# baggepinnen/LPVSpectral.jl

Measured on AMD Instinct MI355X. Metric: signals/sec, ls_sparse_spectral_lpv group lasso N=2^20 Nf=512 Nv=8 (2000 ADMM iters; iters/sec in admm_iters_per_sec), higher is better.
Workload: dtype f64

## Files before the change

### lpvspectral.jl_amd/csrc/api.hip

```cpp
#include <cmath>
#include <cstdarg>
#include <cstdio>
#include <cstdlib>
#include <cstring>
#include <ctime>
#include <map>
#include <mutex>
#include <array>
#include <thread>
#include <string>
#include <vector>

#include "lpvs_internal.h"

namespace lpvs {

static thread_local char g_err[512] = "";

void set_error(const char *fmt, ...) {
    va_list ap;
    va_start(ap, fmt);
    vsnprintf(g_err, sizeof(g_err), fmt, ap);
    va_end(ap);
}
// ... 448 lines not shown

AdmmParams make_params(const lpvs_problem *h) {
    const StoragePlan &pl = h->plan;
    const bool sym = h->np >= kSymmetricMinNp;
    AdmmParams p{h->M.as<double>(), h->np, h->n, h->bs.as<double>(), h->x.as<double>(), h->z.as<double>(), h->u.as<double>(),
                 h->rhs.as<double>(), h->mu, h->tol, h->prox_kind, h->prox_param, h->group_len, h->status.as<AdmmStatus>(),
                 h->scratch.as<double>(), h->part.as<double>(), sym ? h->Mp.as<double>() : nullptr, (int)h->ns};
    p.mp_f32 = pl.mode == kMpF32 ? 1 : 0;
    p.mp_split = pl.mode == kMpSplit || pl.mode == kMpMixed ? 1 : 0;
    p.mp_types = pl.mode == kMpMixed ? mp_tile_types(h->Mp, h->np, 1) : nullptr;
    p.mp_fix32 = p.mp_types != nullptr && (pl.fix_bits <= 32 || pl.nib_period > 0) ? 1 : 0;
    p.nib_period = pl.nib_period; p.nib_ramp = pl.nib_ramp; p.xb_corr = h->xb_corr.as<double>(); p.nib_rhs = h->nib_rhs.as<double>(); p.nib_part = h->nib_part.as<double>(); p.nib_acc = h->nib_acc.as<long long>();
    p.xb = pl.offset_form ? h->xb.as<double>() : nullptr;
    p.fi = pl.owns_fi && h->fi.p ? h->fi.as<double>() : nullptr;
    p.fi_R = h->fi_R; p.fi_xbmax = h->fi_xbmax;
    p.fi_prefetch_all = pl.mode == kMpMixed && h->Mp_census.fixed == h->Mp_census.total ? 1 : 0;
    p.opt_iteration = h->opt[LPVS_OPT_ITERATION]; p.opt_nt_loads = h->opt[LPVS_OPT_NT_LOADS];
    {
        const char *e = experiment_env("LPVS_TILE_ORDER");
        p.tile_order = p.fi != nullptr && !(e && std::string(e) == "forward") ? 1 : 0;
    }
    p.sm_ctl = !sym && h->sm_ctl.p ? h->sm_ctl.as<int>() : nullptr;
    p.prox_params = h->prox_per_signal && h->ns > 1 ? h->prox_params.as<double>() : nullptr;
    return p;
}

int32_t factorize(lpvs_problem *h, double shift) {
    if (h->M_valid && h->M_shift == shift) return LPVS_OK;
    const int64_t np = h->np, n = h->n;
    h->Mp_valid = false; h->Mp_rowsum = 0;
    if (!h->M.p) LPVS_TRY(h->M.alloc(sizeof(double) * (size_t)np * (size_t)np));
    if (!h->work.p) LPVS_TRY(h->work.alloc(spd_inverse_work_bytes(np)));
    LPVS_HIP(hipEventRecord(h->ev[3].a, h->stream));
    LPVS_HIP(hipMemcpyAsync(h->M.p, h->G.p, sizeof(double) * (size_t)np * (size_t)np, hipMemcpyDeviceToDevice, h->stream));
    LPVS_TRY(launch_add_diag(h->M.as<double>(), np, n, shift, h->stream));
    LPVS_TRY(spd_inverse_inplace(h->M.as<double>(), np, h->work.as<double>(), h->istat.as<int>(), h->stream, &h->res->aux));
    LPVS_HIP(hipEventRecord(h->ev[3].b, h->stream));
    int st = 0;
    LPVS_HIP(hipMemcpyAsync(&st, h->istat.p, sizeof(int), hipMemcpyDeviceToHost, h->stream));
    LPVS_HIP(hipStreamSynchronize(h->stream));
    h->t_factor += h->ev[3].ms();
    if (st != 0) {
        h->M_valid = false;
        set_error("(G + %.3g I) is not positive definite (non-positive pivot in the block sweep)", shift);
        return LPVS_ENUMERIC;
    }
    h->M_valid = true; h->M_shift = shift;
    return LPVS_OK;
}


StoragePlan decide_plan(lpvs_problem *h) {
    const int xc_opt = option_in_effect(LPVS_OPT_XUPDATE_CORRECTION, h->opt[LPVS_OPT_XUPDATE_CORRECTION]);
    const bool corrected = h->np >= kSymmetricMinNp && xc_opt != LPVS_XCORR_OFF;
    h->xcorr = xcorr_schedule_from(corrected ? experiment_env("LPVS_XUPDATE_CORRECTION") : nullptr, xcorr_default_schedule(h->ns, corrected));
    const int storage = option_in_effect(LPVS_OPT_M_STORAGE, h->opt[LPVS_OPT_M_STORAGE]);
    return admm_storage_plan(h->np, h->ns, h->f32, storage, h->ns > 1 && multi_signal_fixed_tiles_ok(h->np), h->xcorr.on(), fix_bits_from(experiment_env),
                             nib_knobs_from(experiment_env));
}

int32_t pack_mixed(lpvs_problem *h, const StoragePlan &want, StoragePlan *stored) {
    hipStream_t s = h->stream;
    const PackedLayout lay = packed_layout(h->np, want.element_bytes, 1);
    unsigned char *types = mp_tile_types(h->Mp, h->np, 1);
    unsigned long long *amax = reinterpret_cast<unsigned long long *>(h->Mp.as<unsigned char>() + lay.absmax_off);
    LPVS_TRY(launch_pack_tiles_mixed(h->M.as<double>(), h->np, h->Mp.as<unsigned char>(), types, amax, s, want.diag_float,
                                     want.want_rowsum ? h->part.as<double>() : nullptr, h->n, want.want_rowsum ? h->scratch.as<double>() : nullptr, want.fix_bits));
    std::vector<unsigned char> ht(lay.tiles);
// ... 2786 lines not shown
```

### lpvspectral.jl_amd/csrc/linalg.hip

```cpp
#include "lpvs_internal.h"
#include "factor_plan.h"

#include <cstdlib>
#include <map>
#include <mutex>
#include <string>
#include <vector>

namespace lpvs {

namespace {

typedef double f64x4 __attribute__((ext_vector_type(4)));
constexpr int NB = 64;

__global__ void __launch_bounds__(256)
diag_inverse_kernel(const double *__restrict__ Aall, int64_t np, int k, double *__restrict__ Pall, int *status,
                    int64_t strideA, int64_t strideW) {
    __shared__ double colp[NB], rowp[NB];
    const double *A = Aall + (int64_t)blockIdx.x * strideA;
    double *P = Pall + (int64_t)blockIdx.x * strideW;
    const double *blk = A + (int64_t)k * NB * np + (int64_t)k * NB;
    const int ti = threadIdx.x >> 4, tj = threadIdx.x & 15;
    double v[4][4];
#pragma unroll
    for (int a = 0; a < 4; ++a)
#pragma unroll
        for (int b = 0; b < 4; ++b) {
            const int i = 4 * ti + a, j = 4 * tj + b;
            v[a][b] = j <= i ? blk[(int64_t)i * np + j] : blk[(int64_t)j * np + i];
        }
    for (int pb = 0; pb < NB / 4; ++pb) {
#pragma unroll
        for (int pp = 0; pp < 4; ++pp) {
// ... 623 lines not shown
            S[li * KWF + (c ^ (2 * li))] = acc[b][rg];
        }
    __syncthreads();
#pragma unroll
    for (int i = 0; i < KWF * RS / 256; ++i) {
        const int e = tid + 256 * i, r = e >> 7, c = e & 127;
        A[(R0 + r) * np + k0 + c] = S[r * KWF + (c ^ (2 * r))];
    }
}

constexpr int kMaxGroup = 4;
struct RuGroup {
    const double *Ck[kMaxGroup], *Bk[kMaxGroup];
    int kb, mg;
};
template <int BK, int WGS>
__global__ void __launch_bounds__(RU_THREADS, WGS)
rank_updatem_kernel(double *__restrict__ A, int64_t np, int64_t ldp, RuGroup g, const int2 *__restrict__ tiles, int ntiles,
                    int select, int e0, int nslices, int band, int skip0, int nskip) {
    extern __shared__ __attribute__((aligned(16))) double lds[];
    const int tid = threadIdx.x, lane = tid & 63;
    const int wave = __builtin_amdgcn_readfirstlane(tid >> 6);
    const int wa = wave / RU_WN, wb = wave % RU_WN;
    int2 tt;
    if (select == 1) {
        const int nr = (int)(np / RU_TM);
        const int bsl = blockIdx.x / nr, e = blockIdx.x - bsl * nr, bt = e0 + bsl;
        if (e > bt && e < e0 + nslices) return;
        tt = e <= bt ? make_int2(bt, e) : make_int2(e, bt);
    } else {
        const int bq = ntiles / 8, br = ntiles % 8, xcd = blockIdx.x % 8, bm = blockIdx.x / 8;
        const int item = (xcd < br ? xcd * (bq + 1) : br * (bq + 1) + (xcd - br) * bq) + bm;
        tt = tiles[item];
        if ((tt.x >= skip0 && tt.x < skip0 + nskip) || (tt.y >= skip0 && tt.y < skip0 + nskip)) return;
    }
    const int jr = (tt.x >= g.kb && tt.x < g.kb + g.mg) ? tt.x - g.kb : -1, jc = (tt.y >= g.kb && tt.y < g.kb + g.mg) ? tt.y - g.kb : -1;
    int lo, hi;
    if (band >= 0) { lo = (jc >= 0 && jc < band) ? jc + 1 : 0; hi = band; }
    else { lo = (jr > jc ? jr : jc) + 1; hi = g.mg; }
    if (lo >= hi) return;
    const int64_t a0 = (int64_t)tt.x * RU_TM, b0 = (int64_t)tt.y * RU_TN;
    const int64_t r_lo = a0 + wa * 64, c_lo = b0 + wb * 64;
    const bool skip_wave = c_lo > r_lo + 63 || c_lo >= np;
    constexpr int SPP = 128 / BK;
    const int nstages = (hi - lo) * SPP;

    constexpr int ROW = RU_TM + RU_TN, STAGE = BK * ROW;
    double *buf0 = lds, *buf1 = lds + STAGE;
    auto stage_load = [&](double *buf, int st) {
        const int pi = lo + st / SPP, s0 = (st % SPP) * BK;
        const double *Ck = nullptr, *Bk = nullptr;
#pragma unroll
        for (int i = 0; i < kMaxGroup; ++i) if (i == pi) { Ck = g.Ck[i]; Bk = g.Bk[i]; }
        for (int p = wave; p < BK * 2; p += RU_THREADS / 64) {
            const int k = p >> 1, part = p & 1;
            const double *src = part == 0 ? Ck + (int64_t)(s0 + k) * ldp + a0 : Bk + (int64_t)(s0 + k) * ldp + b0;
            glds16(src + 2 * lane, buf + p * 128);
        }
    };
    const int li = lane & 15, lk = lane >> 4;
    int offA[4], offB[4];
#pragma unroll
    for (int t = 0; t < 4; ++t) { offA[t] = wa * 64 + t * 16 + li; offB[t] = RU_TM + wb * 64 + t * 16 + li; }
    stage_load(buf0, 0);
    f64x4 acc[4][4];
    const unsigned voffb = (unsigned)((lk * np + li) * 8);
    const bool below = c_lo + 63 <= r_lo;
    if (!skip_wave && below) {
#pragma unroll
        for (int i = 0; i < 4; ++i)
#pragma unroll
            for (int r = 0; r < 4; ++r) {
// ... 49 lines not shown
        for (int i = 0; i < 4; ++i)
#pragma unroll
            for (int r = 0; r < 4; ++r) {
                double *sp = A + (r_lo + i * 16 + 4 * r) * np + c_lo;
#pragma unroll
                for (int j = 0; j < 4; ++j) *reinterpret_cast<double *>(reinterpret_cast<char *>(sp + j * 16) + voffb) = acc[i][j][r];
            }
        return;
    }
#pragma unroll
    for (int i = 0; i < 4; ++i)
#pragma unroll
        for (int j = 0; j < 4; ++j)
#pragma unroll
            for (int r = 0; r < 4; ++r) {
                const int64_t row = r_lo + i * 16 + lk + 4 * r, col = c_lo + j * 16 + li;
                if (col <= row) A[row * np + col] = acc[i][j][r];
            }
}

template <int BK>
__global__ void __launch_bounds__(256, 4)
rank_updateb_kernel(double *__restrict__ A, int64_t np, int64_t ldp, RuGroup g, int e0, int nslices, int band) {
    extern __shared__ __attribute__((aligned(16))) double lds[];
    const int tid = threadIdx.x, lane = tid & 63;
    const int wave = __builtin_amdgcn_readfirstlane(tid >> 6);
    const int wa = wave >> 1, wb = wave & 1;
    const int sub = blockIdx.x & 3, bidx = blockIdx.x >> 2, sx = sub >> 1, sy = sub & 1;
    const int nr = (int)(np / 128);
    const int bsl = bidx / nr, e = bidx - bsl * nr, bt = e0 + bsl;
    if (e > bt && e < e0 + nslices) return;
    const int2 tt = e <= bt ? make_int2(bt, e) : make_int2(e, bt);
    if (tt.x == tt.y && sy > sx) return;
    const int jr = (tt.x >= g.kb && tt.x < g.kb + g.mg) ? tt.x - g.kb : -1, jc = (tt.y >= g.kb && tt.y < g.kb + g.mg) ? tt.y - g.kb : -1;
    int lo, hi;
    if (band >= 0) { lo = (jc >= 0 && jc < band) ? jc + 1 : 0; hi = band; }
    else { lo = (jr > jc ? jr : jc) + 1; hi = g.mg; }
    if (lo >= hi) return;
    const int64_t a0 = (int64_t)tt.x * 128 + sx * 64, b0 = (int64_t)tt.y * 128 + sy * 64;
    const int64_t r_lo = a0 + wa * 32, c_lo = b0 + wb * 32;
    const bool skip_wave = c_lo > r_lo + 31;
    constexpr int SPP = 128 / BK;
    const int nstages = (hi - lo) * SPP;
    constexpr int ROW = 128, STAGE = BK * ROW;
    double *buf0 = lds, *buf1 = lds + STAGE;
    auto stage_load = [&](double *buf, int st) {
        const int pi = lo + st / SPP, s0 = (st % SPP) * BK;
        const double *Ck = nullptr, *Bk = nullptr;
#pragma unroll
        for (int i = 0; i < kMaxGroup; ++i) if (i == pi) { Ck = g.Ck[i]; Bk = g.Bk[i]; }
        for (int k = wave; k < BK; k += 4) {
            const double *src = lane < 32 ? Ck + (int64_t)(s0 + k) * ldp + a0 + 2 * lane : Bk + (int64_t)(s0 + k) * ldp + b0 + 2 * (lane - 32);
            glds16(src, buf + k * ROW);
        }
    };
    const int li = lane & 15, lk = lane >> 4;
    int offA[2], offB[2];
#pragma unroll
    for (int t = 0; t < 2; ++t) { offA[t] = wa * 32 + t * 16 + li; offB[t] = 64 + wb * 32 + t * 16 + li; }
    stage_load(buf0, 0);
    f64x4 acc[2][2];
    const unsigned voffb = (unsigned)((lk * np + li) * 8);
    const bool below = c_lo + 31 <= r_lo;
    if (!skip_wave && below) {
#pragma unroll
        for (int i = 0; i < 2; ++i)
#pragma unroll
            for (int r = 0; r < 4; ++r) {
                const double *sp = A + (r_lo + i * 16 + 4 * r) * np + c_lo;
#pragma unroll
// ... 38 lines not shown
                        acc[i][j] = __builtin_amdgcn_mfma_f64_16x16x4f64(opA[i], opB[j], acc[i][j], 0, 0, 0);
                __builtin_amdgcn_sched_barrier(0);
            }
        }
        __syncthreads();
    }
    if (skip_wave) return;
    if (below) {
#pragma unroll
        for (int i = 0; i < 2; ++i)
#pragma unroll
            for (int r = 0; r < 4; ++r) {
                double *sp = A + (r_lo + i * 16 + 4 * r) * np + c_lo;
#pragma unroll
                for (int j = 0; j < 2; ++j) *reinterpret_cast<double *>(reinterpret_cast<char *>(sp + j * 16) + voffb) = acc[i][j][r];
            }
        return;
    }
#pragma unroll
    for (int i = 0; i < 2; ++i)
#pragma unroll
        for (int j = 0; j < 2; ++j)
#pragma unroll
            for (int r = 0; r < 4; ++r) {
                const int64_t row = r_lo + i * 16 + lk + 4 * r, col = c_lo + j * 16 + li;
                if (col <= row) A[row * np + col] = acc[i][j][r];
            }
}

__global__ void __launch_bounds__(256) add_diag_kernel(double *__restrict__ Mall, int64_t np, int64_t n, double shift) {
    const int64_t i = (int64_t)blockIdx.x * 256 + threadIdx.x;
    double *M = Mall + (int64_t)blockIdx.y * np * np;
    if (i < np) M[i * np + i] = i < n ? M[i * np + i] + shift : 1.0;
}

__global__ void __launch_bounds__(256) negate_mirror_kernel(double *__restrict__ Aall, int64_t np) {
    __shared__ double tile[32][33];
    double *A = Aall + (int64_t)blockIdx.z * np * np;
    const int bi = blockIdx.y, bj = blockIdx.x;
    if (bj > bi) return;
    const int tx = threadIdx.x & 31, ty = threadIdx.x >> 5;
    const int64_t r0 = (int64_t)bi * 32, c0 = (int64_t)bj * 32;
    for (int r = ty; r < 32; r += 8) {
        const double v = -A[(r0 + r) * np + c0 + tx];
        tile[r][tx] = v;
        if (bi != bj || tx <= r) A[(r0 + r) * np + c0 + tx] = v;
    }
    __syncthreads();
    for (int r = ty; r < 32; r += 8)
        if (bi != bj || tx > r) A[(c0 + r) * np + r0 + tx] = tile[tx][r];
}

__global__ void __launch_bounds__(256)
symm_matmul_kernel(const double *__restrict__ A, const double *__restrict__ B, double *__restrict__ C, int64_t np) {
    const int lane = threadIdx.x & 63, wave = threadIdx.x >> 6;
    const int64_t r0 = ((int64_t)blockIdx.y * 2 + (wave >> 1)) * 64, c0 = ((int64_t)blockIdx.x * 2 + (wave & 1)) * 64;
    const int li = lane & 15, lk = lane >> 4;
    f64x4 acc[4][4];
#pragma unroll
    for (int i = 0; i < 4; ++i)
#pragma unroll
        for (int j = 0; j < 4; ++j) acc[i][j] = (f64x4){0.0, 0.0, 0.0, 0.0};
    for (int64_t kk = 0; kk < np; kk += 4) {
        double opA[4], opB[4];
#pragma unroll
        for (int q = 0; q < 4; ++q) {
// ... 37 lines not shown
        if (two > d) d = two;
    }
    return sizeof(double) * d;
}

static void sweep64(double *A, int64_t np, int nbatch, double *work, int *status_dev, hipStream_t s) {
    const int64_t strideW = (int64_t)sweep64_work_doubles(np), strideA = np * np;
    double *Bp = work, *Cp = work + np * NB, *P = work + 2 * np * NB;
    const int nblk = (int)(np / NB);
    const int nt = (int)(np / 128);
    const unsigned ntiles = (unsigned)(nt * (nt + 1) / 2);
    for (int k = 0; k < nblk; ++k) {
        hipLaunchKernelGGL(diag_inverse_kernel, dim3((unsigned)nbatch), dim3(256), 0, s, A, np, k, P, status_dev, strideA, strideW);
        hipLaunchKernelGGL(panel_kernel, dim3((unsigned)nblk, (unsigned)nbatch), dim3(256), 0, s, A, np, k, P, Bp, Cp, strideA, strideW);
        hipLaunchKernelGGL(sweep_update_kernel, dim3(ntiles, (unsigned)nbatch), dim3(256), 0, s, A, np, k, Bp, Cp, strideA, strideW);
    }
}

static const std::vector<int2> &ru_tiles(int64_t np) {
    static std::mutex mu;
    static std::map<int64_t, std::vector<int2>> cache;
    std::lock_guard<std::mutex> g(mu);
    auto it = cache.find(np);
    if (it != cache.end()) return it->second;
    std::vector<int2> t;
    const int nr = (int)(np / RU_TM), nc = (int)ceil_div(np, RU_TN);
    for (int band = 0; band < nr; band += 4)
        for (int tj = 0; tj < nc; ++tj)
            for (int ti = band; ti < band + 4 && ti < nr; ++ti)
                if ((int64_t)tj * RU_TN <= (int64_t)ti * RU_TM + RU_TM - 1) t.push_back(make_int2(ti, tj));
    return cache.emplace(np, std::move(t)).first->second;
}

int32_t SweepAux::ensure() {
    if (side) return LPVS_OK;
    int lo = 0, hi = 0;
    LPVS_HIP(hipDeviceGetStreamPriorityRange(&lo, &hi));
    LPVS_HIP(hipStreamCreateWithPriority(&side, hipStreamNonBlocking, hi));
    LPVS_HIP(hipEventCreateWithFlags(&panel, hipEventDisableTiming));
    LPVS_HIP(hipEventCreateWithFlags(&rest, hipEventDisableTiming));
    LPVS_HIP(hipEventCreateWithFlags(&band, hipEventDisableTiming));
    LPVS_HIP(hipEventCreateWithFlags(&second, hipEventDisableTiming));
    LPVS_HIP(hipEventCreateWithFlags(&bulkdone, hipEventDisableTiming));
    const int o_res = option_in_effect(LPVS_OPT_RESERVE_CUS);
    const int reserve = o_res == LPVS_RESERVE_NONE ? 0 : (o_res > 0 ? o_res : 8);
    int dev = 0, cus = 0;
    if (reserve > 0 && hipGetDevice(&dev) == hipSuccess && hipDeviceGetAttribute(&cus, hipDeviceAttributeMultiprocessorCount, dev) == hipSuccess &&
        cus > 4 * reserve) {
        std::vector<uint32_t> mask((size_t)(cus + 31) / 32, 0u);
        for (int c = reserve; c < cus; ++c) mask[(size_t)c / 32] |= 1u << (c % 32);
        if (hipExtStreamCreateWithCUMask(&bulk, (uint32_t)mask.size(), mask.data()) != hipSuccess) { (void)hipGetLastError(); bulk = nullptr; }
    }
    return LPVS_OK;
}
SweepAux::~SweepAux() {
    if (side) { (void)hipStreamSynchronize(side); (void)hipStreamDestroy(side); }
    if (bulk) { (void)hipStreamSynchronize(bulk); (void)hipStreamDestroy(bulk); }
    if (bulkdone) (void)hipEventDestroy(bulkdone);
    if (panel) (void)hipEventDestroy(panel);
    if (rest) (void)hipEventDestroy(rest);
    if (band) (void)hipEventDestroy(band);
    if (second) (void)hipEventDestroy(second);
}


struct FactorCtx {
    double *A;
    int64_t np, ldp;
    double *panels, *P, *inner;
    int2 *tiles;
    int ntiles;
    int *status_dev;
    hipStream_t s;
    SweepAux *aux;
    double *stepB(int i) const { return panels + i * kStepPairRows * ldp; }
    double *stepC(int i) const { return stepB(i) + KW * ldp; }
    double *slotB(int blk) const { return panels + (int64_t)(blk & (kGroupSlots - 1)) * (kGroupSlotRows * ldp); }
    double *slotC(int blk) const { return slotB(blk) + 128 * ldp; }
};

constexpr size_t kRuLds = sizeof(double) * 2 * RU_BK * (RU_TM + RU_TN);

static int step_width(const FactorCtx &c, const FactorPlan &plan, int64_t k0) {
    return (int)(c.np - k0 < plan.kw_outer ? c.np - k0 : plan.kw_outer);
}

static void step_chain(const FactorCtx &c, const FactorPlan &plan, int64_t k0, double *Bk, double *Ck, hipStream_t st) {
    const int kw = step_width(c, plan, k0);
    if (plan.pivot == PivotKernel::regs && kw == 128) {
        hipLaunchKernelGGL(pivot_inverse_kernel<128>, dim3(1), dim3(192), 0, st, c.A, c.np, k0, c.P, c.status_dev);
    } else {
// ... 108 lines not shown
}

static void group_chain(const FactorCtx &c, const FactorPlan &plan, const GroupKernels &k, int blk, hipStream_t st) {
    const int64_t k0 = (int64_t)blk * 128;
    if (plan.pivot == PivotKernel::mfma) hipLaunchKernelGGL(pivot_inverse_mfma_kernel, dim3(1), dim3(256), k.pivot_pad, st, c.A, c.np, k0, c.P, c.status_dev);
    else hipLaunchKernelGGL(pivot_inverse_kernel<128>, dim3(1), dim3(192), 0, st, c.A, c.np, k0, c.P, c.status_dev);
    if (plan.fused_chain) {
        hipLaunchKernelGGL(panel_fused_kernel, dim3((unsigned)(c.ldp / 16)), dim3(256), 0, st, c.A, c.np, c.ldp, k0, (const double *)c.P, c.slotB(blk), c.slotC(blk));
    } else {
        hipLaunchKernelGGL(panel_gather_kernel, dim3((unsigned)(c.ldp / 64)), dim3(256), 0, st, c.A, c.np, c.ldp, k0, 128, c.slotB(blk));
        hipLaunchKernelGGL(panel_gemm_kernel, dim3((unsigned)(c.ldp / 64)), dim3(256), 0, st, c.A, c.np, c.ldp, k0, 128, c.P, c.slotB(blk), c.slotC(blk));
    }
}

static RuGroup group_of(const FactorCtx &c, int kb, int mg) {
    RuGroup g{};
    for (int i = 0; i < kMaxGroup; ++i) { g.Ck[i] = c.slotC(kb + (i < mg ? i : 0)); g.Bk[i] = c.slotB(kb + (i < mg ? i : 0)); }
    g.kb = kb; g.mg = mg;
    return g;
}

static void group_bands(const FactorCtx &c, const FactorPlan &plan, const GroupKernels &k, hipStream_t st, const RuGroup &g, int e0, int nsl, int band) {
    const int nr = (int)(c.np / RU_TM);
    if (plan.band_tile == 64)
        hipLaunchKernelGGL(rank_updateb_kernel<16>, dim3((unsigned)(4 * nr * nsl)), dim3(256), 2 * 16 * 128 * sizeof(double), st, c.A, c.np, c.ldp, g, e0, nsl, band);
    else
        hipLaunchKernelGGL(k.ru_kernel, dim3((unsigned)(nr * nsl)), dim3(RU_THREADS), k.ru_lds, st, c.A, c.np, c.ldp, g, c.tiles, c.ntiles, 1, e0, nsl, band, 0, 0);
}

static void group_rest(const FactorCtx &c, const GroupKernels &k, hipStream_t st, const RuGroup &g, int skip0, int nskip) {
    hipLaunchKernelGGL(k.ru_kernel, dim3((unsigned)c.ntiles), dim3(RU_THREADS), k.ru_lds, st, c.A, c.np, c.ldp, g, c.tiles, c.ntiles, 0, 0, 0, -1, skip0, nskip);
}

static int32_t factor_groups(const FactorCtx &c, const FactorPlan &plan) {
    GroupKernels k{};
    LPVS_TRY(group_kernels(c, plan, k));
    SweepAux *aux = c.aux;
    hipStream_t s = c.s, side = aux->side;
    hipStream_t mb = aux->bulk ? aux->bulk : s;
    const int nblocks = (int)(c.np / 128), mgmax = plan.group_max;
    LPVS_HIP(hipEventRecord(aux->rest, s));
    LPVS_HIP(hipStreamWaitEvent(side, aux->rest, 0));
    if (mb != s) LPVS_HIP(hipStreamWaitEvent(mb, aux->rest, 0));
    group_chain(c, plan, k, 0, side);
    bool rest_pending = false;
    for (int kb = 0; kb < nblocks;) {
        const int mg = nblocks - kb < mgmax ? nblocks - kb : mgmax, nb0 = kb + mg;
        const int mgn = nblocks - nb0 < mgmax ? nblocks - nb0 : mgmax;
        const RuGroup g = group_of(c, kb, mg);
        for (int j = 1; j < mg; ++j) {
            group_bands(c, plan, k, side, g, kb + j, 1, j);
            group_chain(c, plan, k, kb + j, side);
        }
        LPVS_HIP(hipEventRecord(aux->panel, side));
        LPVS_HIP(hipStreamWaitEvent(mb, aux->panel, 0));
        group_rest(c, k, mb, g, nb0, mgn);
        if (mgn > 0) {
            if (rest_pending) LPVS_HIP(hipStreamWaitEvent(side, aux->second, 0));
            group_bands(c, plan, k, side, g, nb0, mgn, -1);
            group_chain(c, plan, k, nb0, side);
        }
        LPVS_HIP(hipEventRecord(aux->second, mb));
        rest_pending = true;
        LPVS_HIP(hipGetLastError());
        kb = nb0;
    }
    if (mb != s) {
        LPVS_HIP(hipEventRecord(aux->bulkdone, mb));
        LPVS_HIP(hipStreamWaitEvent(s, aux->bulkdone, 0));
    }
    LPVS_HIP(hipEventRecord(aux->rest, side));
    LPVS_HIP(hipStreamWaitEvent(s, aux->rest, 0));
    return LPVS_OK;
}

static int32_t spd_inverse_two_level(double *A, int64_t np, double *work, int *status_dev, hipStream_t s, SweepAux *aux, const FactorPlan &plan) {
    FactorCtx c{};
    c.A = A; c.np = np; c.ldp = round_up(np, RU_TN);
    c.panels = work; c.P = work + kPanelRows * c.ldp; c.inner = c.P + KW * KW;
    c.tiles = reinterpret_cast<int2 *>(c.inner + sweep64_work_doubles(KW));
    c.status_dev = status_dev; c.s = s; c.aux = aux;
    const std::vector<int2> &ht = ru_tiles(np);
    c.ntiles = (int)ht.size();
    LPVS_HIP(hipMemcpyAsync(c.tiles, ht.data(), sizeof(int2) * ht.size(), hipMemcpyHostToDevice, s));
    LPVS_HIP(hipFuncSetAttribute(reinterpret_cast<const void *>(&rank_update_kernel), hipFuncAttributeMaxDynamicSharedMemorySize, (int)kRuLds));
    if (plan.schedule != FactorSchedule::steps_serial) LPVS_TRY(aux->ensure());
    switch (plan.schedule) {
    case FactorSchedule::groups: return factor_groups(c, plan);
    case FactorSchedule::steps_depth2: return factor_steps_depth2(c, plan);
    case FactorSchedule::steps_depth1: return factor_steps_depth1(c, plan);
    case FactorSchedule::steps_serial: break;
    }
    return factor_steps_serial(c, plan);
}

static int32_t spd_inverse_impl(double *A, int64_t np, int nbatch, double *work, int *status_dev, hipStream_t s, SweepAux *aux) {
    if (np % 128 != 0) { set_error("spd_inverse: np=%lld not a multiple of 128", (long long)np); return LPVS_ESTATE; }
    LPVS_HIP(hipMemsetAsync(status_dev, 0, sizeof(int) * (size_t)nbatch, s));
    const FactorPlan plan = factor_plan(np, nbatch, aux != nullptr, factor_knobs_from(experiment_env));
    if (plan.level == FactorLevel::two) {
        LPVS_TRY(spd_inverse_two_level(A, np, work, status_dev, s, aux, plan));
    } else {
        sweep64(A, np, nbatch, work, status_dev, s);
        LPVS_HIP(hipGetLastError());
    }
    hipLaunchKernelGGL(negate_mirror_kernel, dim3((unsigned)(np / 32), (unsigned)(np / 32), (unsigned)nbatch), dim3(256), 0, s, A, np);
    LPVS_HIP(hipGetLastError());
    return LPVS_OK;
}

int32_t spd_inverse_inplace_batch(double *A, int64_t np, int nbatch, double *work, int *status_dev, hipStream_t s) {
    return spd_inverse_impl(A, np, nbatch, work, status_dev, s, nullptr);
}

int32_t spd_inverse_inplace(double *A, int64_t np, double *work, int *status_dev, hipStream_t s, SweepAux *aux) {
    return spd_inverse_impl(A, np, 1, work, status_dev, s, aux);
}

int32_t launch_add_diag_batch(double *M, int64_t np, int64_t n, double shift, int nbatch, hipStream_t s) {
    hipLaunchKernelGGL(add_diag_kernel, dim3((unsigned)ceil_div(np, 256), (unsigned)nbatch), dim3(256), 0, s, M, np, n, shift);
    LPVS_HIP(hipGetLastError());
    return LPVS_OK;
}

int32_t launch_add_diag(double *M, int64_t np, int64_t n, double shift, hipStream_t s) {
    hipLaunchKernelGGL(add_diag_kernel, dim3((unsigned)ceil_div(np, 256)), dim3(256), 0, s, M, np, n, shift);
    LPVS_HIP(hipGetLastError());
    return LPVS_OK;
}

int32_t launch_symm_matmul(const double *A, const double *B, double *C, int64_t np, hipStream_t s) {
    if (np % 128 != 0) return LPVS_ESTATE;
    hipLaunchKernelGGL(symm_matmul_kernel, dim3((unsigned)(np / 128), (unsigned)(np / 128)), dim3(256), 0, s, A, B, C, np);
    LPVS_HIP(hipGetLastError());
    return LPVS_OK;
}

}
```

### lpvspectral.jl_amd/csrc/lpvs_internal.h

```cpp
#pragma once
#include <hip/hip_runtime.h>
#include <exception>
#include <new>
#include <stdint.h>
#include <functional>
#include <string>
#include <vector>

#include "../../include/lpvspectral.h"
#include "windows_plan.h"
#include "admm_plan.h"
#include "gram_form_plan.h"
#include "eval_plan.h"
#include "lomb_plan.h"
#include "lomb_boot_plan.h"
#include "lomb_terms_plan.h"
#include "wwz_plan.h"

namespace lpvs {

inline const char *experiment_env(const char *name) {
#ifdef LPVS_NO_EXPERIMENTS
    (void)name;
    return nullptr;
// ... 192 lines not shown
int32_t launch_lomb_boot_moments(const double *y, const double *w, int64_t N, int64_t seed, int64_t row0, int64_t B, bool center, double *mean, double *mom,
                                 hipStream_t s);
int32_t launch_lomb_boot_sums(const double *t, const double *w, const double *y, int64_t N, int64_t seed, int64_t row0, int64_t r0, int64_t count,
                              const double *mean_or_null, const double *f_dev, int64_t Nf, const LombBootPlan &plan, double *part, double *sums, hipStream_t s);
int32_t launch_lomb_boot_epilogue(const double *shared, const double *sums, int64_t Nf, int64_t r0, int64_t count, const double *mean, const double *mom,
                                  bool fit_mean, bool center, bool psd, int64_t N, double *power_or_null, double *maxv, int64_t *maxi, bool count_deg, int *ndeg_dev,
                                  hipStream_t s);

int32_t launch_lomb_terms_sums(const double *t, const double *w, const double *wy, int64_t N, int64_t ns, const double *f_dev, int64_t Nf, const LombTermsPlan &pl,
                               double *part, double *sums, hipStream_t s);
int32_t launch_lomb_terms_epilogue(int K, const double *sums, int64_t Nf, int64_t ns, const double *mom_dev, const double *mean_dev, bool fit_mean, bool center,
                                   bool psd, int64_t N, double *power, double *coef, int *ndeg_dev, hipStream_t s);

struct WwzArgs {
    const double *t = nullptr, *y = nullptr, *W = nullptr;
    const double *mean = nullptr;
    const double *f = nullptr, *decay = nullptr, *radius = nullptr;
    const double *tau = nullptr;
    const int32_t *pos = nullptr;
    const WwzItem *items = nullptr;
    const int64_t *offset = nullptr, *first_slab = nullptr;
    int64_t N = 0, Nf = 0, Ntau = 0, nitems = 0, ftiles = 0, slab_samples = 0, rows = 0;
    int ns = 0, TT = 0;
};
int32_t launch_wwz_sorted(const double *t, int64_t N, int *flags_dev, hipStream_t s);
int32_t launch_wwz_ranges(const double *t, int64_t N, const double *a, const double *b, int64_t na, const double *r, int64_t nr, int64_t *edges, hipStream_t s);
int32_t launch_wwz_sums(const WwzArgs &A, int ts, double *part, hipStream_t s);
int32_t launch_wwz_epilogue(const WwzArgs &A, const double *part, const int64_t *cell_edges, bool center, double *power, double *amplitude, double *wwz,
                            double *neff, double *coef, int64_t *count_out, int32_t *empty_out, int *flags_dev, unsigned long long *counters, hipStream_t s);

struct SweepAux {
    hipStream_t side = nullptr;
    hipStream_t bulk = nullptr;
    hipEvent_t panel = nullptr, rest = nullptr, band = nullptr, second = nullptr, bulkdone = nullptr;
    int32_t ensure();
    ~SweepAux();
};
size_t spd_inverse_work_bytes(int64_t np);
int32_t spd_inverse_inplace(double *A, int64_t np, double *work, int *status_dev, hipStream_t s, SweepAux *aux = nullptr);
int32_t launch_add_diag(double *M, int64_t np, int64_t n, double shift, hipStream_t s);
int32_t launch_add_diag_batch(double *M, int64_t np, int64_t n, double shift, int nbatch, hipStream_t s);
int32_t spd_inverse_inplace_batch(double *A, int64_t np, int nbatch, double *work, int *status_dev, hipStream_t s);
int32_t launch_symm_matmul(const double *A, const double *B, double *C, int64_t np, hipStream_t s);

struct AdmmStatus {
    long long iters;
    int converged;
    int pad;
    double nxz;
};
struct AdmmParams {
    const double *M;
    int64_t np;
    int64_t n;
    const double *b;
    double *x, *z, *u, *rhs;
    double mu, tol;
    int prox_kind;
    double prox_param;
    int64_t group_len;
    AdmmStatus *status;
    double *scratch;
    double *part;
    const double *Mp;
    int ns;
    int mp_f32 = 0;
    int mp_split = 0;
    int nib_period = 0;
    int nib_ramp = 0;
    int mp_fix32 = 0;
    const double *xb_corr = nullptr;
    double *nib_rhs = nullptr;
// ... 125 lines not shown
```

Before: 15.52.

## Restructure blocked SPD inverse group schedule with deferred multi-stream updates

Moves the grouped factorization's issue loop into a schedule generator. Under an experiment flag it processes pairs of groups, splitting trailing updates into priority, small, early and deep launches spread over an extra CU-masked bulk stream, to overlap more of the critical panel chain. It also fuses the G-to-M copy and diagonal shift into one kernel that copies only the lower block triangle. The per-call host-to-device upload of the tile list is replaced by a per-device cached buffer. The default path changes the head-start ordering for small np, and the extra events and streams add complexity and race risk.

```diff
diff --git a/lpvspectral.jl_amd/csrc/api.hip b/lpvspectral.jl_amd/csrc/api.hip
--- a/lpvspectral.jl_amd/csrc/api.hip
+++ b/lpvspectral.jl_amd/csrc/api.hip
@@ -504,8 +504,7 @@
     if (!h->M.p) LPVS_TRY(h->M.alloc(sizeof(double) * (size_t)np * (size_t)np));
     if (!h->work.p) LPVS_TRY(h->work.alloc(spd_inverse_work_bytes(np)));
     LPVS_HIP(hipEventRecord(h->ev[3].a, h->stream));
-    LPVS_HIP(hipMemcpyAsync(h->M.p, h->G.p, sizeof(double) * (size_t)np * (size_t)np, hipMemcpyDeviceToDevice, h->stream));
-    LPVS_TRY(launch_add_diag(h->M.as<double>(), np, n, shift, h->stream));
+    LPVS_TRY(launch_copy_lower_shift(h->G.as<double>(), h->M.as<double>(), np, n, shift, h->stream));
     LPVS_TRY(spd_inverse_inplace(h->M.as<double>(), np, h->work.as<double>(), h->istat.as<int>(), h->stream, &h->res->aux));
     LPVS_HIP(hipEventRecord(h->ev[3].b, h->stream));
     int st = 0;
diff --git a/lpvspectral.jl_amd/csrc/factor_defer.h b/lpvspectral.jl_amd/csrc/factor_defer.h
--- /dev/null
+++ b/lpvspectral.jl_amd/csrc/factor_defer.h
@@ -0,0 +1,141 @@
+#pragma once
+
+#if defined(__HIPCC__)
+#define LPVS_FACTOR_DEFER_HD __host__ __device__
+#else
+#define LPVS_FACTOR_DEFER_HD
+#endif
+
+namespace lpvs {
+
+constexpr int kDeferMaxPanels = 4;
+constexpr int kDeferSlots = 8;
+
+struct PanelSpan { int lo, hi; };
+
+LPVS_FACTOR_DEFER_HD inline bool in_blocks(int b, int b0, int n) { return b >= b0 && b < b0 + n; }
+
+LPVS_FACTOR_DEFER_HD inline PanelSpan update_panels(int tr, int tc, int kb, int mg, int band) {
+    const int jr = in_blocks(tr, kb, mg) ? tr - kb : -1, jc = in_blocks(tc, kb, mg) ? tc - kb : -1;
+    PanelSpan p;
+    if (band >= 0) { p.lo = (jc >= 0 && jc < band) ? jc + 1 : 0; p.hi = band; }
+    else { p.lo = (jr > jc ? jr : jc) + 1; p.hi = mg; }
+    return p;
+}
+
+LPVS_FACTOR_DEFER_HD inline bool update_skips(int tr, int tc, int skip0, int nskip) { return in_blocks(tr, skip0, nskip) || in_blocks(tc, skip0, nskip); }
+
+enum class GroupStream { side, deep, early };
+enum class GroupEvent { panel, second, early, small };
+enum class UpdateKind {
+    band,
+    priority,
+    rest,
+    small,
+    early,
+    deep
+};
+struct UpdateLaunch {
+    UpdateKind kind;
+    int kb, mg;
+    int e0, nsl;
+    int band;
+    int skip0, nskip;
+    LPVS_FACTOR_DEFER_HD bool direct() const { return kind != UpdateKind::rest && kind != UpdateKind::deep; }
+    LPVS_FACTOR_DEFER_HD bool covers(int tr, int tc) const {
+        if (direct() && !(in_blocks(tr, e0, nsl) || in_blocks(tc, e0, nsl))) return false;
+        return !update_skips(tr, tc, skip0, nskip);
+    }
+    LPVS_FACTOR_DEFER_HD PanelSpan panels(int tr, int tc) const { return update_panels(tr, tc, kb, mg, band); }
+};
+
+constexpr long long kHeadStartBelowNp = 8192;
+
+inline int defer_min(int a, int b) { return a < b ? a : b; }
+inline int defer_clamp(int v, int lo, int hi) { return v < lo ? lo : (v > hi ? hi : v); }
+
+inline bool defer_applies(int group_max, bool defer) { return defer && group_max == 2; }
+
+template <class V>
+void group_schedule(int nblocks, int group_max, bool defer, bool head, V &v) {
+    const bool pairs = defer_applies(group_max, defer);
+    bool rest_pending = false, early_pending = false;
+    for (int kb = 0; kb < nblocks;) {
+        if (pairs && kb % 4 == 0 && kb + 4 <= nblocks) {
+            const int a = kb, after = nblocks - (a + 4);
+            const int n_small = defer_clamp(after, 0, 2), n_early = defer_clamp(after - 2, 0, 4), n_skip = defer_clamp(after, 0, 6);
+            const auto priority_odd = [&] {
+                v.update(GroupStream::side, UpdateLaunch{UpdateKind::priority, a, 2, a + 2, 2, -1, 0, 0});
+                v.chain(a + 2);
+            };
+            const auto priority_next = [&] {
+                v.update(GroupStream::side, UpdateLaunch{UpdateKind::priority, a + 2, 2, a + 4, n_small, -1, 0, 0});
+                v.chain(a + 4);
+            };
+            v.update(GroupStream::side, UpdateLaunch{UpdateKind::band, a, 2, a + 1, 1, 1, 0, 0});
+            v.chain(a + 1);
+            if (head && early_pending) v.wait(GroupStream::side, GroupEvent::early);
+            v.record(GroupEvent::panel, GroupStream::side);
+            if (head) priority_odd();
+            if (n_small > 0) {
+                v.wait(GroupStream::early, GroupEvent::panel);
+                v.update(GroupStream::early, UpdateLaunch{UpdateKind::small, a, 2, a + 4, n_small, -1, a + 2, 2});
+                v.record(GroupEvent::small, GroupStream::early);
+            }
+            if (!head) {
+                if (early_pending) v.wait(GroupStream::side, GroupEvent::early);
+                priority_odd();
+            }
+            v.update(GroupStream::side, UpdateLaunch{UpdateKind::band, a + 2, 2, a + 3, 1, 1, 0, 0});
+            v.chain(a + 3);
+            if (head) {
+                if (rest_pending) v.wait(GroupStream::side, GroupEvent::second);
+                if (n_small > 0) v.wait(GroupStream::side, GroupEvent::small);
+            }
+            v.record(GroupEvent::panel, GroupStream::side);
+            if (head && n_small > 0) priority_next();
+            if (!head && rest_pending) v.wait(GroupStream::side, GroupEvent::second);
+            if (n_early > 0) {
+                v.wait(GroupStream::early, GroupEvent::panel);
+                if (!head && rest_pending) v.wait(GroupStream::early, GroupEvent::second);
+                v.update(GroupStream::early, UpdateLaunch{UpdateKind::early, a, 4, a + 6, n_early, -1, a + 4, 2});
+                v.record(GroupEvent::early, GroupStream::early);
+                early_pending = true;
+            }
+            v.wait(GroupStream::deep, GroupEvent::panel);
+            v.update(GroupStream::deep, UpdateLaunch{UpdateKind::deep, a, 4, 0, 0, -1, a + 4, n_skip});
+            v.record(GroupEvent::second, GroupStream::deep);
+            rest_pending = true;
+            if (!head && n_small > 0) {
+                v.wait(GroupStream::side, GroupEvent::small);
+                priority_next();
+            }
+            kb = a + 4;
+            continue;
+        }
+        const int mg = defer_min(nblocks - kb, group_max), nb0 = kb + mg, mgn = defer_min(nblocks - nb0, group_max);
+        const auto side_waits = [&] {
+            if (rest_pending) v.wait(GroupStream::side, GroupEvent::second);
+            if (early_pending) { v.wait(GroupStream::side, GroupEvent::early); early_pending = false; }
+        };
+        const auto priority_next = [&] {
+            v.update(GroupStream::side, UpdateLaunch{UpdateKind::priority, kb, mg, nb0, mgn, -1, 0, 0});
+            v.chain(nb0);
+        };
+        for (int j = 1; j < mg; ++j) {
+            v.update(GroupStream::side, UpdateLaunch{UpdateKind::band, kb, mg, kb + j, 1, j, 0, 0});
+            v.chain(kb + j);
+        }
+        if (head && mgn > 0) side_waits();
+        v.record(GroupEvent::panel, GroupStream::side);
+        if (head && mgn > 0) priority_next();
+        v.wait(GroupStream::deep, GroupEvent::panel);
+        v.update(GroupStream::deep, UpdateLaunch{UpdateKind::rest, kb, mg, 0, 0, -1, nb0, mgn});
+        if (!head && mgn > 0) { side_waits(); priority_next(); }
+        v.record(GroupEvent::second, GroupStream::deep);
+        rest_pending = true;
+        kb = nb0;
+    }
+}
+
+}
diff --git a/lpvspectral.jl_amd/csrc/linalg.hip b/lpvspectral.jl_amd/csrc/linalg.hip
--- a/lpvspectral.jl_amd/csrc/linalg.hip
+++ b/lpvspectral.jl_amd/csrc/linalg.hip
@@ -1,5 +1,6 @@
 #include "lpvs_internal.h"
 #include "factor_plan.h"
+#include "factor_defer.h"
 
 #include <cstdlib>
 #include <map>
@@ -689,12 +690,10 @@
         const int bq = ntiles / 8, br = ntiles % 8, xcd = blockIdx.x % 8, bm = blockIdx.x / 8;
         const int item = (xcd < br ? xcd * (bq + 1) : br * (bq + 1) + (xcd - br) * bq) + bm;
         tt = tiles[item];
-        if ((tt.x >= skip0 && tt.x < skip0 + nskip) || (tt.y >= skip0 && tt.y < skip0 + nskip)) return;
-    }
-    const int jr = (tt.x >= g.kb && tt.x < g.kb + g.mg) ? tt.x - g.kb : -1, jc = (tt.y >= g.kb && tt.y < g.kb + g.mg) ? tt.y - g.kb : -1;
-    int lo, hi;
-    if (band >= 0) { lo = (jc >= 0 && jc < band) ? jc + 1 : 0; hi = band; }
-    else { lo = (jr > jc ? jr : jc) + 1; hi = g.mg; }
+    }
+    if (update_skips(tt.x, tt.y, skip0, nskip)) return;
+    const PanelSpan span = update_panels(tt.x, tt.y, g.kb, g.mg, band);
+    const int lo = span.lo, hi = span.hi;
     if (lo >= hi) return;
     const int64_t a0 = (int64_t)tt.x * RU_TM, b0 = (int64_t)tt.y * RU_TN;
     const int64_t r_lo = a0 + wa * 64, c_lo = b0 + wb * 64;
@@ -810,10 +809,8 @@
     if (e > bt && e < e0 + nslices) return;
     const int2 tt = e <= bt ? make_int2(bt, e) : make_int2(e, bt);
     if (tt.x == tt.y && sy > sx) return;
-    const int jr = (tt.x >= g.kb && tt.x < g.kb + g.mg) ? tt.x - g.kb : -1, jc = (tt.y >= g.kb && tt.y < g.kb + g.mg) ? tt.y - g.kb : -1;
-    int lo, hi;
-    if (band >= 0) { lo = (jc >= 0 && jc < band) ? jc + 1 : 0; hi = band; }
-    else { lo = (jr > jc ? jr : jc) + 1; hi = g.mg; }
+    const PanelSpan span = update_panels(tt.x, tt.y, g.kb, g.mg, band);
+    const int lo = span.lo, hi = span.hi;
     if (lo >= hi) return;
     const int64_t a0 = (int64_t)tt.x * 128 + sx * 64, b0 = (int64_t)tt.y * 128 + sy * 64;
     const int64_t r_lo = a0 + wa * 32, c_lo = b0 + wb * 32;
@@ -918,6 +915,18 @@
     const int64_t i = (int64_t)blockIdx.x * 256 + threadIdx.x;
     double *M = Mall + (int64_t)blockIdx.y * np * np;
     if (i < np) M[i * np + i] = i < n ? M[i * np + i] + shift : 1.0;
+}
+
+__global__ void __launch_bounds__(256)
+copy_lower_shift_kernel(const double *__restrict__ G, double *__restrict__ M, int64_t np, int64_t n, double shift) {
+    const int I = blockIdx.y, J = blockIdx.x;
+    if (J > (I | 1)) return;
+    const int64_t col = (int64_t)J * 128 + (threadIdx.x & 127);
+    for (int r = threadIdx.x >> 7; r < 128; r += 2) {
+        const int64_t row = (int64_t)I * 128 + r;
+        const double v = G[row * np + col];
+        M[row * np + col] = row != col ? v : (row < n ? v + shift : 1.0);
+    }
 }
 
 __global__ void __launch_bounds__(256) negate_mirror_kernel(double *__restrict__ Aall, int64_t np) {
@@ -1021,6 +1030,26 @@
     return cache.emplace(np, std::move(t)).first->second;
 }
 
+static int32_t ru_tiles_device(int64_t np, int2 **tiles, int *ntiles) {
+    static std::mutex mu;
+    static std::map<std::pair<int, int64_t>, int2 *> cache;
+    const std::vector<int2> &ht = ru_tiles(np);
+    *ntiles = (int)ht.size();
+    int dev = 0;
+    LPVS_HIP(hipGetDevice(&dev));
+    std::lock_guard<std::mutex> g(mu);
+    auto it = cache.find({dev, np});
+    if (it == cache.end()) {
+        int2 *d = nullptr;
+        LPVS_HIP(hipMalloc(reinterpret_cast<void **>(&d), sizeof(int2) * ht.size()));
+        const hipError_t e = hipMemcpy(d, ht.data(), sizeof(int2) * ht.size(), hipMemcpyHostToDevice);
+        if (e != hipSuccess) { (void)hipFree(d); LPVS_HIP(e); }
+        it = cache.emplace(std::make_pair(dev, np), d).first;
+    }
+    *tiles = it->second;
+    return LPVS_OK;
+}
+
 int32_t SweepAux::ensure() {
     if (side) return LPVS_OK;
     int lo = 0, hi = 0;
@@ -1031,6 +1060,8 @@
     LPVS_HIP(hipEventCreateWithFlags(&band, hipEventDisableTiming));
     LPVS_HIP(hipEventCreateWithFlags(&second, hipEventDisableTiming));
     LPVS_HIP(hipEventCreateWithFlags(&bulkdone, hipEventDisableTiming));
+    LPVS_HIP(hipEventCreateWithFlags(&early, hipEventDisableTiming));
+    LPVS_HIP(hipEventCreateWithFlags(&small, hipEventDisableTiming));
     const int o_res = option_in_effect(LPVS_OPT_RESERVE_CUS);
     const int reserve = o_res == LPVS_RESERVE_NONE ? 0 : (o_res > 0 ? o_res : 8);
     int dev = 0, cus = 0;
@@ -1039,13 +1070,22 @@
         std::vector<uint32_t> mask((size_t)(cus + 31) / 32, 0u);
         for (int c = reserve; c < cus; ++c) mask[(size_t)c / 32] |= 1u << (c % 32);
         if (hipExtStreamCreateWithCUMask(&bulk, (uint32_t)mask.size(), mask.data()) != hipSuccess) { (void)hipGetLastError(); bulk = nullptr; }
-    }
+        if (bulk) bulk_mask = mask;
+    }
+    return LPVS_OK;
+}
+int32_t SweepAux::ensure_bulk2() {
+    if (bulk2 || !bulk) return LPVS_OK;
+    if (hipExtStreamCreateWithCUMask(&bulk2, (uint32_t)bulk_mask.size(), bulk_mask.data()) != hipSuccess) { (void)hipGetLastError(); bulk2 = nullptr; }
     return LPVS_OK;
 }
 SweepAux::~SweepAux() {
     if (side) { (void)hipStreamSynchronize(side); (void)hipStreamDestroy(side); }
     if (bulk) { (void)hipStreamSynchronize(bulk); (void)hipStreamDestroy(bulk); }
+    if (bulk2) { (void)hipStreamSynchronize(bulk2); (void)hipStreamDestroy(bulk2); }
     if (bulkdone) (void)hipEventDestroy(bulkdone);
+    if (early) (void)hipEventDestroy(early);
+    if (small) (void)hipEventDestroy(small);
     if (panel) (void)hipEventDestroy(panel);
     if (rest) (void)hipEventDestroy(rest);
     if (band) (void)hipEventDestroy(band);
@@ -1220,38 +1260,49 @@
     hipLaunchKernelGGL(k.ru_kernel, dim3((unsigned)c.ntiles), dim3(RU_THREADS), k.ru_lds, st, c.A, c.np, c.ldp, g, c.tiles, c.ntiles, 0, 0, 0, -1, skip0, nskip);
 }
 
+struct GroupIssuer {
+    const FactorCtx &c;
+    const FactorPlan &plan;
+    const GroupKernels &k;
+    hipStream_t streams[3];
+    hipEvent_t events[4];
+    hipError_t err = hipSuccess;
+    void chain(int blk) { if (err == hipSuccess) { group_chain(c, plan, k, blk, streams[(int)GroupStream::side]); err = hipGetLastError(); } }
+    void update(GroupStream on, const UpdateLaunch &u) {
+        if (err != hipSuccess) return;
+        hipStream_t st = streams[(int)on];
+        const RuGroup g = group_of(c, u.kb, u.mg);
+        if (u.kind == UpdateKind::band || u.kind == UpdateKind::priority) group_bands(c, plan, k, st, g, u.e0, u.nsl, u.band);
+        else if (u.direct()) hipLaunchKernelGGL(k.ru_kernel, dim3((unsigned)(c.np / RU_TM * u.nsl)), dim3(RU_THREADS), k.ru_lds, st, c.A, c.np, c.ldp, g, c.tiles, c.ntiles, 1, u.e0, u.nsl, -1, u.skip0, u.nskip);
+        else group_rest(c, k, st, g, u.skip0, u.nskip);
+        err = hipGetLastError();
+    }
+    void record(GroupEvent e, GroupStream on) { if (err == hipSuccess) err = hipEventRecord(events[(int)e], streams[(int)on]); }
+    void wait(GroupStream on, GroupEvent e) { if (err == hipSuccess) err = hipStreamWaitEvent(streams[(int)on], events[(int)e], 0); }
+};
+
 static int32_t factor_groups(const FactorCtx &c, const FactorPlan &plan) {
     GroupKernels k{};
     LPVS_TRY(group_kernels(c, plan, k));
     SweepAux *aux = c.aux;
     hipStream_t s = c.s, side = aux->side;
     hipStream_t mb = aux->bulk ? aux->bulk : s;
-    const int nblocks = (int)(c.np / 128), mgmax = plan.group_max;
+    const char *kd = experiment_env("LPVS_FACTOR_DEFER"), *kh = experiment_env("LPVS_FACTOR_HEAD");
+    const bool defer = kd && kd[0] == '1';
+    const bool head = kh ? kh[0] != '0' : (defer || c.np < kHeadStartBelowNp);
+    if (defer_applies(plan.group_max, defer)) LPVS_TRY(aux->ensure_bulk2());
+    hipStream_t eb = defer && aux->bulk2 ? aux->bulk2 : mb;
     LPVS_HIP(hipEventRecord(aux->rest, s));
     LPVS_HIP(hipStreamWaitEvent(side, aux->rest, 0));
     if (mb != s) LPVS_HIP(hipStreamWaitEvent(mb, aux->rest, 0));
+    if (eb != mb) LPVS_HIP(hipStreamWaitEvent(eb, aux->rest, 0));
     group_chain(c, plan, k, 0, side);
-    bool rest_pending = false;
-    for (int kb = 0; kb < nblocks;) {
-        const int mg = nblocks - kb < mgmax ? nblocks - kb : mgmax, nb0 = kb + mg;
-        const int mgn = nblocks - nb0 < mgmax ? nblocks - nb0 : mgmax;
-        const RuGroup g = group_of(c, kb, mg);
-        for (int j = 1; j < mg; ++j) {
-            group_bands(c, plan, k, side, g, kb + j, 1, j);
-            group_chain(c, plan, k, kb + j, side);
-        }
-        LPVS_HIP(hipEventRecord(aux->panel, side));
-        LPVS_HIP(hipStreamWaitEvent(mb, aux->panel, 0));
-        group_rest(c, k, mb, g, nb0, mgn);
-        if (mgn > 0) {
-            if (rest_pending) LPVS_HIP(hipStreamWaitEvent(side, aux->second, 0));
-            group_bands(c, plan, k, side, g, nb0, mgn, -1);
-            group_chain(c, plan, k, nb0, side);
-        }
-        LPVS_HIP(hipEventRecord(aux->second, mb));
-        rest_pending = true;
-        LPVS_HIP(hipGetLastError());
-        kb = nb0;
+    GroupIssuer v{c, plan, k, {side, mb, eb}, {aux->panel, aux->second, aux->early, aux->small}};
+    group_schedule((int)(c.np / 128), plan.group_max, defer, head, v);
+    LPVS_HIP(v.err);
+    if (eb != mb) {
+        LPVS_HIP(hipEventRecord(aux->early, eb));
+        LPVS_HIP(hipStreamWaitEvent(s, aux->early, 0));
     }
     if (mb != s) {
         LPVS_HIP(hipEventRecord(aux->bulkdone, mb));
@@ -1266,11 +1317,8 @@
     FactorCtx c{};
     c.A = A; c.np = np; c.ldp = round_up(np, RU_TN);
     c.panels = work; c.P = work + kPanelRows * c.ldp; c.inner = c.P + KW * KW;
-    c.tiles = reinterpret_cast<int2 *>(c.inner + sweep64_work_doubles(KW));
     c.status_dev = status_dev; c.s = s; c.aux = aux;
-    const std::vector<int2> &ht = ru_tiles(np);
-    c.ntiles = (int)ht.size();
-    LPVS_HIP(hipMemcpyAsync(c.tiles, ht.data(), sizeof(int2) * ht.size(), hipMemcpyHostToDevice, s));
+    LPVS_TRY(ru_tiles_device(np, &c.tiles, &c.ntiles));
     LPVS_HIP(hipFuncSetAttribute(reinterpret_cast<const void *>(&rank_update_kernel), hipFuncAttributeMaxDynamicSharedMemorySize, (int)kRuLds));
     if (plan.schedule != FactorSchedule::steps_serial) LPVS_TRY(aux->ensure());
     switch (plan.schedule) {
@@ -1311,6 +1359,13 @@
     return LPVS_OK;
 }
 
+int32_t launch_copy_lower_shift(const double *G, double *M, int64_t np, int64_t n, double shift, hipStream_t s) {
+    if (np % 128 != 0) { set_error("copy_lower_shift: np=%lld not a multiple of 128", (long long)np); return LPVS_ESTATE; }
+    hipLaunchKernelGGL(copy_lower_shift_kernel, dim3((unsigned)(np / 128), (unsigned)(np / 128)), dim3(256), 0, s, G, M, np, n, shift);
+    LPVS_HIP(hipGetLastError());
+    return LPVS_OK;
+}
+
 int32_t launch_add_diag(double *M, int64_t np, int64_t n, double shift, hipStream_t s) {
     hipLaunchKernelGGL(add_diag_kernel, dim3((unsigned)ceil_div(np, 256)), dim3(256), 0, s, M, np, n, shift);
     LPVS_HIP(hipGetLastError());
diff --git a/lpvspectral.jl_amd/csrc/lpvs_internal.h b/lpvspectral.jl_amd/csrc/lpvs_internal.h
--- a/lpvspectral.jl_amd/csrc/lpvs_internal.h
+++ b/lpvspectral.jl_amd/csrc/lpvs_internal.h
@@ -248,12 +248,17 @@
 struct SweepAux {
     hipStream_t side = nullptr;
     hipStream_t bulk = nullptr;
+    hipStream_t bulk2 = nullptr;
+    std::vector<uint32_t> bulk_mask;
+    int32_t ensure_bulk2();
     hipEvent_t panel = nullptr, rest = nullptr, band = nullptr, second = nullptr, bulkdone = nullptr;
+    hipEvent_t early = nullptr, small = nullptr;
     int32_t ensure();
     ~SweepAux();
 };
 size_t spd_inverse_work_bytes(int64_t np);
 int32_t spd_inverse_inplace(double *A, int64_t np, double *work, int *status_dev, hipStream_t s, SweepAux *aux = nullptr);
+int32_t launch_copy_lower_shift(const double *G, double *M, int64_t np, int64_t n, double shift, hipStream_t s);
 int32_t launch_add_diag(double *M, int64_t np, int64_t n, double shift, hipStream_t s);
 int32_t launch_add_diag_batch(double *M, int64_t np, int64_t n, double shift, int nbatch, hipStream_t s);
 int32_t spd_inverse_inplace_batch(double *A, int64_t np, int nbatch, double *work, int *status_dev, hipStream_t s);
```

Result: no change. 15.40 (-0.8%).
